# sevagh/umx.cpp

Hardware: AMD Instinct MI355X
Metric: realtime-factor (audio-sec/wall-sec) UMX-L 4-stem, 60 s seg (higher is better)
Workload: dtype f32 (activations as 2 x fp16 planes of the power-of-two-scaled row, integer weights exact in fp16, f32 accumulate on the fp16 matrix cores; fp32-grade: 1.4-2.2x the error of an fp32 evaluation, profiles/r06_v2_accuracy_vs_float64.txt)

## Files before the change

umx.cpp_amd/csrc/engine.hip:

```cpp
#include "../../include/umx_hip.h"
#include <chrono>
#include <dlfcn.h>

#include <algorithm>
#include <numeric>
#include <cmath>
#include <cstdio>
#include <cstdlib>
#include <cstring>
#include <map>
#include <mutex>
#include <string>
#include <vector>

#include "common.h"
#include "gemm_bf16x3.h"
#include "gemm_planes.h"
#include "gemm_planes_pp.h"
#include "gemm_planes_ps.h"
#include "lstm_kernels.h"
#include "lstm_batch.h"
#include "lstm_batch8.h"
#include "track_kernels.h"
#include "resample.h"
// ... 104 lines not shown
{
    static const RoctxApi api;
    if (!api.push)
        return;
    if (t_stage_range_open)
        api.pop();
    t_stage_range_open = stage >= 0 && stage < ST_COUNT;
    if (t_stage_range_open)
        api.push(api.names[stage]);
}
struct StageRangeCloser
{
    ~StageRangeCloser() { stage_range(-1); }
};
}

struct Lane
{
    TargetAct ta[4];
    float2 *spec = nullptr, *y = nullptr, *frames = nullptr;
    float *x = nullptr, *wpart = nullptr, *Rc = nullptr;
    unsigned *maxabs = nullptr;
};

struct Slot
{
    hipStream_t stream = nullptr;
    Lane lane[LSTMB_MAX_TRACKS];
    float *hbuf = nullptr;
    float *wv = nullptr;
    bool lstm_wrote_planes[3] = {false, false, false};
    bool lstm_rows_f32[3] = {true, true, true};
    unsigned *status = nullptr, *lsync = nullptr;
    unsigned long long *lprof = nullptr;
    hipEvent_t ev[ST_COUNT + 1] = {};
    hipEvent_t evk[ST_COUNT] = {};
    bool evk_set[ST_COUNT] = {};
    hipEvent_t rec_done[3] = {};
    hipEvent_t k_done = nullptr;
    hipEvent_t out_free = nullptr;
    bool out_free_valid = false;
    bool have_times = false, last_persistent = false, used = false;
};
}

namespace
{
struct LstmGate
{
    std::mutex m;
    struct Grid
    {
        hipEvent_t done;
        int units;
        hipStream_t stream;
        unsigned long long seq;
    };
    std::vector<Grid> inflight;
    std::vector<hipEvent_t> pool;
    unsigned long long seq = 0;
    int reserved = 0;
    std::vector<int> reservations;
};
LstmGate g_gate[16];

template <class Launch> hipError_t lstm_gate_launch(int device, hipStream_t st, int units, int capacity_units, Launch launch)
// ... 212 lines not shown
            slot[si].used = false;
    }
    int B = 1;
    bool lstm_batched = false;
    unsigned tag_epoch = 0;
    unsigned next_tag_base()
    {
        tag_epoch = (tag_epoch + 1) & 0xFFFFF;
        return tag_epoch << 12;
    }
    int cur = 0;
    long long nseg = 0;
    size_t lsync_words = 0;
    bool persistent_ok = true;
    int n_cus = 256;
    struct PendingCall
    {
        int nb;
        const float *audio[LSTMB_MAX_TRACKS];
        int n[LSTMB_MAX_TRACKS];
        float *out[4 * LSTMB_MAX_TRACKS];
        float *host_out[4 * LSTMB_MAX_TRACKS];
        const float *host_audio[LSTMB_MAX_TRACKS];
        unsigned flags;
    };
    static constexpr int kBackupCalls = 8;
    std::vector<PendingCall> pending;
    bool pending_lost = false;
    float *backup = nullptr;
    bool no_recovery = false, recovering = false;
    int recover();
    int lstm_poll_delay = 0;
    int env_gemm_ps = -1;
    int env_gemm_pp = -1;
    const char *gemm_kernel_last[4] = {"none", "none", "none", "none"};
    const char *lstm_kernel_last = "none";
    int lstm_capacity = 0;
    unsigned last_flags = 0;
    hipStream_t stream = nullptr;

    void set_error(const std::string &s) { err = s; }

    template <class T_> int dalloc(T_ **p, size_t count, bool zero = true)
    {
        void *q = nullptr;
        UMX_HIP_CHECK(hipMalloc(&q, std::max<size_t>(count, 1) * sizeof(T_)));
        allocs.push_back(q);
        if (zero)
            UMX_HIP_CHECK(hipMemset(q, 0, std::max<size_t>(count, 1) * sizeof(T_)));
        *p = reinterpret_cast<T_ *>(q);
        return UMX_OK;
    }
    template <class T_> int upload(T_ **p, const std::vector<T_> &h)
    {
        int rc = dalloc(p, h.size(), false);
        if (rc)
            return rc;
        UMX_HIP_CHECK(hipMemcpy(*p, h.data(), h.size() * sizeof(T_), hipMemcpyHostToDevice));
        return UMX_OK;
    }
    int init(int device_, int hidden, int segment_samples, const umx_tensor_view *tensors, int n_tensors,
             unsigned create_flags, int n_tracks);
    size_t weight_bytes = 0;
    bool wiener_fused = true;
    bool gemm_planes = false;
    void launch_split(Lane &ln, int nl, hipStream_t st, int which, const int *active, int nact);
    void launch_gemm_planes(Lane &ln, int nl, hipStream_t st, int mode, int layer, const int *active, int nact, bool dbg);
    void launch_gemm_lanes(Slot &sl, hipStream_t st, int nb, const float *const *audio_dev, int mode, int layer, const int *active,
                           int nact, bool dbg);
    bool u8_dequant = false;
    unsigned char *whh_q[3] = {};
    float whh_s[3][8] = {}, whh_o[3][8] = {};
    int infer_device(const float *audio_dev, int n, float *const out[4], unsigned flags);
    int infer_batch(int nb, const float *const *audio_dev, const int *n, float *const *out , unsigned flags);
    int lstm_batch_capacity = 0;
    bool lstm_batch8_ok = false;
    int lstm8_poll_delay = 0;
    bool env_lstm8_paired = true;
    int env_lstm8_min = 1;
    bool lstm_rowsums = false;
    bool lstm_writes_planes = false;
    size_t state_floats() const { return (size_t)4 * 12 * Hl; }
    struct TrackRequest
    {
        int n_tracks = 0;
        const float *const *audio = nullptr;
        const int *length = nullptr;
        const int *rate = nullptr;
        const int *shift_offset = nullptr;
        float *const *out = nullptr;
        unsigned flags = 0;
        void (*progress)(float, void *) = nullptr;
        void *progress_user = nullptr;
        bool ensemble = false;
        const MixSpec *mix = nullptr;
    };
    int tracks(const TrackRequest &rq);
    int tracks_once(const TrackRequest &rq);
    std::map<std::pair<int, int>, float *> rs_taps;
    int resample_plan(int rate_in, int rate_out, ResampleGeom &g, const float **taps_dev);
// ... 148 lines not shown
```

umx.cpp_amd/csrc/engine_init.h:

```cpp
namespace
{
bool dequant(const umx_tensor_view &tv, size_t expect, std::vector<float> &out)
{
    size_t nel = 1;
    for (int i = 0; i < tv.n_dims; ++i)
        nel *= (size_t)tv.ne[i];
    if (nel != expect)
        return false;
    out.resize(nel);
    if (tv.dtype == UMX_DTYPE_F32)
        memcpy(out.data(), tv.data, nel * sizeof(float));
    else if (tv.dtype == UMX_DTYPE_U8)
    {
        const uint8_t *q = static_cast<const uint8_t *>(tv.data);
        for (size_t i = 0; i < nel; ++i)
            out[i] = (float)q[i] * tv.scale + tv.offset;
    }
    else if (tv.dtype == UMX_DTYPE_U16)
    {
        const uint16_t *q = static_cast<const uint16_t *>(tv.data);
        for (size_t i = 0; i < nel; ++i)
            out[i] = (float)q[i] * tv.scale + tv.offset;
    }
    else
// ... 67 lines not shown
            return false;
        }
        return true;
    };

    const bool keepq = !(create_flags & UMX_CREATE_DEQUANTISE_AT_LOAD);
    auto view = [&](int tg, const std::string &name) -> const umx_tensor_view * {
        auto it = idx[tg].find(name);
        return it == idx[tg].end() ? nullptr : it->second;
    };
    auto all_q = [&](const std::string &name, int dtype, size_t expect) {
        for (int tg = 0; tg < 4; ++tg)
        {
            const umx_tensor_view *tv = view(tg, name);
            size_t n = 1;
            for (int i = 0; tv && i < tv->n_dims; ++i)
                n *= (size_t)tv->ne[i];
            if (!keepq || !tv || tv->dtype != dtype || n != expect)
                return false;
        }
        return true;
    };

    if (create_flags & UMX_CREATE_GEMM_F32)
    {
        set_error("UMX_CREATE_GEMM_F32: the fp32-MFMA GEMM flavour was removed in round 3 (slower and, against float64, less accurate "
                  "than the split-operand kernels: profiles/r02_accuracy_vs_float64.txt)");
        return UMX_ERR_ARG;
    }
    if (const char *e = getenv("UMX_GEMM_PP"))
        env_gemm_pp = atoi(e);
    if (const char *e = getenv("UMX_GEMM_PS"))
        env_gemm_ps = atoi(e);
    if (const char *e = getenv("UMX_LSTM8_POLL_DELAY"))
        lstm8_poll_delay = atoi(e);
    if (const char *e = getenv("UMX_LSTM8_PAIRED"))
        env_lstm8_paired = atoi(e) != 0;
    if (const char *e = getenv("UMX_LSTM8_MIN_LANES"))
        env_lstm8_min = atoi(e);
    if (const char *e = getenv("UMX_LSTM_POLL_DELAY"))
        lstm_poll_delay = atoi(e);
    wiener_fused = lstm_batched;
    if (const char *e = getenv("UMX_WIENER"))
        wiener_fused = std::string(e) == "fused";
    gemm_planes = (create_flags & UMX_CREATE_GEMM_PLANES) || (lstm_batched && !(create_flags & UMX_CREATE_GEMM_STAGED));
    Tp = gemm_planes ? std::max(T, 256) : round_up(T, 128);

    const int G = 4 * Hl;
    std::vector<int> gate_row(G);
    for (int sl = 0; sl < S; ++sl)
        for (int g = 0; g < 4; ++g)
            for (int u = 0; u < 16; ++u)
                gate_row[g * Hl + sl * 16 + u] = sl * 64 + u * 4 + g;
    std::vector<int> fc3_row(NOUT);
    for (int r = 0; r < NOUT; ++r)
        fc3_row[r] = r / NBINS * MAGP + r % NBINS;
    struct WeightDesc
    {
        std::string name[2];
        int nsrc, rows, cols, dst_rows, cols_pad;
        const std::vector<int> *dst_row;
        int dtype;
    };
    WeightDesc wd[W_COUNT];
    wd[W_FC1] = {{"fc1.weight"}, 1, H, NIN, H, KX, nullptr, UMX_DTYPE_U8};
    for (int l = 0; l < 3; ++l)
// ... 348 lines not shown
            }
        }
        {
            const WienerStrides ls = lane_strides();
            float2 *spec_all, *y_all, *frames_all;
            float *wpart_all, *Rc_all;
            unsigned *maxabs_all;
            if (int rc = dalloc(&spec_all, (size_t)B * ls.spec))
                return rc;
            if (int rc = dalloc(&y_all, (size_t)B * ls.y))
                return rc;
            if (int rc = dalloc(&frames_all, (size_t)B * ls.frames))
                return rc;
            if (int rc = dalloc(&wpart_all, (size_t)B * ls.part))
                return rc;
            if (int rc = dalloc(&Rc_all, (size_t)B * ls.rc))
                return rc;
            if (int rc = dalloc(&maxabs_all, (size_t)B))
                return rc;
            for (int ln = 0; ln < B; ++ln)
            {
                Lane &L = sl.lane[ln];
                L.x = x_all + (size_t)ln * Tp * KX;
                L.spec = spec_all + (size_t)ln * ls.spec;
                L.y = y_all + (size_t)ln * ls.y;
                L.frames = frames_all + (size_t)ln * ls.frames;
                L.wpart = wpart_all + (size_t)ln * ls.part;
                L.Rc = Rc_all + (size_t)ln * ls.rc;
                L.maxabs = maxabs_all + ln;
            }
        }
        if (int rc = dalloc(&sl.status, 4))
            return rc;
        if (int rc = dalloc(&sl.hbuf, (size_t)2 * 8 * Hl))
            return rc;
        if (int rc = dalloc(&sl.lsync, lsync_words))
            return rc;
        if (int rc = dalloc(&sl.lprof, 1024 + 64 * 8 * 5))
            return rc;
        for (int i = 0; i <= ST_COUNT; ++i)
            UMX_HIP_CHECK(hipEventCreate(&sl.ev[i]));
        for (int i : {ST_FC1, ST_IH0, ST_IH1, ST_IH2, ST_FC2, ST_FC3})
            UMX_HIP_CHECK(hipEventCreate(&sl.evk[i]));
        for (int l = 0; l < 3; ++l)
            UMX_HIP_CHECK(hipEventCreateWithFlags(&sl.rec_done[l], hipEventDisableTiming));
    }
    stream = slot[0].stream;
    {
        int cus = 0;
        UMX_HIP_CHECK(hipDeviceGetAttribute(&cus, hipDeviceAttributeMultiprocessorCount, device));
        n_cus = cus;
        const bool want8 = lstm_batched && B >= env_lstm8_min && !u8_dequant && whh_q[0] && whh_q[1] && whh_q[2];
        const LstmbLanes ll = lstmb_lanes(B);
        constexpr int kNone = 1 << 30;
        int per_cu[3] = {kNone, kNone, kNone};
        for (const LstmKernel &k : kLstmKernels)
        {
            if (k.hl != Hl || (k.family == LSTM_BATCH && !lstm_batched) || (k.family == LSTM_BATCH8 && !want8))
                continue;
            if (k.lds)
                UMX_HIP_CHECK(hipFuncSetAttribute(k.fn, hipFuncAttributeMaxDynamicSharedMemorySize, (int)k.lds));
            int v = 0;
            UMX_HIP_CHECK(hipOccupancyMaxActiveBlocksPerMultiprocessor(&v, k.fn, LSTM_THREADS, k.family == LSTM_BATCH ? lstmb_lds_bytes(ll.nbp, ll.bulk) : k.lds));
            per_cu[k.family] = std::min(per_cu[k.family], v);
        }
        lstm_capacity = per_cu[LSTM_PERSISTENT] == kNone ? 0 : per_cu[LSTM_PERSISTENT] * cus;
// ... 88 lines not shown
```

umx.cpp_amd/csrc/engine_stages.h:

```cpp
void umx_hip_ctx::launch_gemm(Lane &sl, hipStream_t st, int mode, int layer, const int *active, int nact, bool dbg)
{
    GemmArgs g;
    memset(&g, 0, sizeof g);
    g.M = Tp;
    g.T = T;
    int bq = BQ_F32;
    for (int i = 0; i < nact; ++i)
    {
        const TargetBufs &b = tb[active[i]];
        const TargetAct &c = sl.ta[active[i]];
        const GemmWeight &w = b.w[gemm_weight(mode, layer)];
        GemmTarget &t = g.t[i];
        switch (mode)
        {
        case G_FC1:
            t.A = sl.x; t.C = c.cat;
            t.e0 = b.bn1[0]; t.e1 = b.bn1[1]; t.e2 = b.bn1[2]; t.e3 = b.bn1[3];
            t.q0 = b.in_scale; t.q1 = b.in_mean;
            g.N = H; g.K = KX; g.lda = KX; g.ldc = 2 * H;
            break;
        case G_IH:
            t.A = layer == 0 ? c.cat : layer == 1 ? c.la : c.lb;
            t.C = c.P; t.e0 = b.ih_b[layer];
            g.N = 4 * H; g.K = H; g.lda = layer == 0 ? 2 * H : H; g.ldc = 4 * H;
// ... 51 lines not shown
        case SP_CATR:
            a.src[i] = c.cat + H; a.dst[i] = c.cat_p; a.rowsum[i] = lstm_rowsums ? nullptr : c.rs_catR;
            a.cols = H; a.ld_src = 2 * H; a.ld_dst = 2 * H; a.col0_dst = H; a.plane = rows_all * 2 * H;
            break;
        case SP_LA:
            a.src[i] = c.la; a.dst[i] = c.la_p; a.rowsum[i] = lstm_rowsums ? nullptr : c.rs_la;
            a.cols = H; a.ld_src = H; a.ld_dst = H; a.col0_dst = 0; a.plane = rows_all * H;
            break;
        case SP_LB:
            a.src[i] = c.lb; a.dst[i] = c.lb_p; a.rowsum[i] = lstm_rowsums ? nullptr : c.rs_lb;
            a.cols = H; a.ld_src = H; a.ld_dst = H; a.col0_dst = 0; a.plane = rows_all * H;
            break;
        default:
            a.src[i] = c.a2; a.dst[i] = c.a2_p; a.rowsum[i] = c.rs_a2; a.rowunscale[i] = c.rsc_a2;
            a.cols = H; a.ld_src = H; a.ld_dst = H; a.col0_dst = 0; a.plane = rows_all * H;
            break;
        }
    }
    a.rows_valid = nl * Tp;
    const dim3 grid(round_up(nl * Tp, 256) / 4, 1, nact);
    if (which == SP_XS && a.cols <= 3072)
    {
        hipLaunchKernelGGL(split_planes_shared_kernel<6>, dim3(grid.x), dim3(256), 0, st, a, nact);
        return;
    }
    if (a.cols <= 1024)
        hipLaunchKernelGGL(split_planes_kernel<2>, grid, dim3(256), 0, st, a);
    else if (a.cols <= 3072)
        hipLaunchKernelGGL(split_planes_kernel<6>, grid, dim3(256), 0, st, a);
    else
        hipLaunchKernelGGL(split_planes_kernel<8>, grid, dim3(256), 0, st, a);
}

void umx_hip_ctx::launch_gemm_planes(Lane &ln, int nl, hipStream_t st, int mode, int layer, const int *active, int nact, bool dbg)
{
    GemmPArgs g;
    memset(&g, 0, sizeof g);
    g.M = round_up(nl * Tp, 256);
    g.lanes = nl;
    g.T = T;
    g.Tp_lane = Tp;
    g.mag_lane = (size_t)2 * T * MAGP;
    g.a_unscale = 1.0f / (float)(1 << GP_SPLIT_FIXED_EXP);
    const size_t rows_all = (size_t)B * Tp + Mpad;
    int nbp = 2;
    for (int i = 0; i < nact; ++i)
    {
        const TargetBufs &b = tb[active[i]];
        const TargetAct &c = ln.ta[active[i]];
        const GemmWeight &w = b.w[gemm_weight(mode, layer)];
        GemmPTarget &t = g.t[i];
        t.bsplit = 0x7fffffff;
        switch (mode)
        {
        case G_FC1:
            t.A = c.xs_p; t.C = c.cat; t.rs0 = c.rs_xs; t.rsc = c.rsc_xs;
            t.e0 = b.bn1[0]; t.e1 = b.bn1[1]; t.e2 = b.bn1[2]; t.e3 = b.bn1[3];
            g.N = H; g.K = KX; g.lda = KX; g.ldc = 2 * H; g.a_plane = rows_all * KX;
            break;
        case G_IH:
            t.A = layer == 0 ? c.cat_p : layer == 1 ? c.la_p : c.lb_p;
            t.rs0 = layer == 0 ? c.rs_catL : layer == 1 ? c.rs_la : c.rs_lb;
            if (layer > 0 && lstm_rowsums)
                t.rs1 = t.rs0 + rows_all;
            t.C = c.P; t.e0 = b.ih_b[layer];
            t.bsplit = 2 * H;
            g.N = 4 * H; g.K = H; g.lda = layer == 0 ? 2 * H : H; g.ldc = 4 * H;
            g.a_plane = layer == 0 ? rows_all * 2 * H : rows_all * H;
            break;
        case G_FC2:
            t.A = c.cat_p; t.C = c.a2; t.rs0 = c.rs_catL; t.rs1 = c.rs_catR;
            if (lstm_rowsums)
                t.rs2 = c.rs_catR + rows_all;
            t.e0 = b.bn2[0]; t.e1 = b.bn2[1]; t.e2 = b.bn2[2]; t.e3 = b.bn2[3];
            g.N = H; g.K = 2 * H; g.lda = 2 * H; g.ldc = H; g.a_plane = rows_all * 2 * H;
            break;
        default:
            t.A = c.a2_p; t.C = c.mag; t.rs0 = c.rs_a2; t.rsc = c.rsc_a2;
            t.e0 = b.bn3[0]; t.e1 = b.bn3[1]; t.e2 = b.bn3[2]; t.e3 = b.bn3[3];
            t.q0 = b.out_scale; t.q1 = b.out_mean;
            g.N = NOUT_PAD; g.K = H; g.lda = H; g.ldc = 0; g.a_plane = rows_all * H;
            break;
        }
        t.B = static_cast<const unsigned short *>(w.p);
        t.bs[0] = w.s[0]; t.bs[1] = w.s[1];
        t.bo2[0] = w.o[0]; t.bo2[1] = w.o[1];
        nbp = w.form;
    }
    const int blocks_big = (g.N / 256) * (g.M / 256) * nact;
    const bool big = g.N % 256 == 0 && blocks_big >= 224;
    const int bm = big ? 256 : 128;
    const int gemm_pp = env_gemm_pp;
    const bool pp = big && (gemm_pp < 0 || ((gemm_pp >> mode) & 1));
    const int ps_wgs = n_cus / 8 * 8;
    const bool ps = pp && (env_gemm_ps < 0 || ((env_gemm_ps >> mode) & 1)) && g.K / GP_BK >= 6 && ps_wgs >= 8 && blocks_big > ps_wgs && g.Tp_lane >= 256;
    gemm_kernel_last[mode] = ps ? "gemm_planes_ps_kernel" : pp ? "gemm_planes_pp_kernel" : "gemm_planes_kernel";
    const GemmKernel k = gp_kernel(mode, nbp, ps ? GP_PS : pp ? GP_PP : big ? GP_256 : GP_128);
    void *kargs[] = {&g, &nact};
    if (ps)
        (void)hipLaunchKernel(k.fn, dim3(ps_wgs), dim3(512), kargs, k.lds, st);
    else
        (void)hipLaunchKernel(k.fn, dim3((unsigned)round_up((g.N / bm) * (g.M / bm), 8), 1, nact), dim3(pp ? 512 : big ? 1024 : 256), kargs,
                              k.lds, st);
}

void umx_hip_ctx::launch_gemm_lanes(Slot &sl, hipStream_t st, int nb, const float *const *audio_dev, int mode, int layer,
                                    const int *active, int nact, bool dbg)
{
    if (nact <= 0)
        return;
    for (int l0 = 0; l0 < nb;)
    {
        if (!audio_dev[l0])
        {
            ++l0;
            continue;
        }
        int l1 = l0 + 1;
        while (gemm_planes && l1 < nb && audio_dev[l1])
            ++l1;
        if (gemm_planes)
        {
            const int which = mode == G_FC1 ? SP_XS : mode == G_IH ? (layer == 0 ? SP_CATL : layer == 1 ? SP_LA : SP_LB) : mode == G_FC2 ? SP_CATR : SP_A2;
            const int from_layer = which == SP_LA ? 0 : which == SP_LB ? 1 : which == SP_CATR ? 2 : -1;
            if (from_layer < 0 || !sl.lstm_wrote_planes[from_layer])
                launch_split(sl.lane[l0], l1 - l0, st, which, active, nact);
            {
                const int stg = mode == G_FC1 ? ST_FC1 : mode == G_IH ? ST_IH0 + 2 * layer : mode == G_FC2 ? ST_FC2 : ST_FC3;
                sl.evk_set[stg] = sl.evk[stg] && hipEventRecord(sl.evk[stg], st) == hipSuccess;
            }
            launch_gemm_planes(sl.lane[l0], l1 - l0, st, mode, layer, active, nact, dbg);
        }
        else
            launch_gemm(sl.lane[l0], st, mode, layer, active, nact, dbg);
        l0 = l1;
    }
}

int umx_hip_ctx::stage_front(Slot &sl, hipStream_t st, int nb, const float *const *audio_dev, const int *n, const int *active,
                             int nact)
{
    stage_range(ST_STFT);
    for (int i = 0; i < ST_COUNT; ++i)
        sl.evk_set[i] = false;
    UMX_HIP_CHECK(hipEventRecord(sl.ev[ST_STFT], st));
    {
        StftIn in;
        in.lanes = lane_set(nb, audio_dev);
        for (int i = 0; i < in.lanes.count; ++i)
        {
            in.audio[i] = audio_dev[in.lanes.id[i]];
            in.n[i] = n[in.lanes.id[i]];
        }
        Lane &L0 = sl.lane[0];
        UMX_HIP_CHECK(hipMemsetAsync(L0.maxabs, 0, sizeof(unsigned) * B, st));
        hipLaunchKernelGGL(stft_kernel, dim3((T + STFT_RUN - 1) / STFT_RUN, in.lanes.count), dim3(256), 0, st, in, N, T, window, tw1, tw2, L0.spec, lane_strides().spec, L0.x,
                           (size_t)Tp * KX, L0.maxabs);
    }
    stage_range(ST_FC1);
    UMX_HIP_CHECK(hipEventRecord(sl.ev[ST_FC1], st));
    launch_gemm_lanes(sl, st, nb, audio_dev, G_FC1, 0, active, nact, false);
    stage_range(ST_IH0);
    UMX_HIP_CHECK(hipEventRecord(sl.ev[ST_IH0], st));
    launch_gemm_lanes(sl, st, nb, audio_dev, G_IH, 0, active, nact, false);
// ... 312 lines not shown
```

umx.cpp_amd/csrc/gemm_planes.h:

```cpp
#pragma once
#include "gemm_bf16x3.h"
#include <cmath>
#include <cstring>

namespace umx
{

struct GemmPTarget
{
    const unsigned short *A;
    const unsigned short *B;
    float *C;
    const float *e0, *e1, *e2, *e3, *q0, *q1;
    const float *rs0, *rs1, *rs2;
    const float *rsc;
    float bs[2], bo2[2];
    int bsplit;
};

struct GemmPArgs
{
    GemmPTarget t[4];
    int M, N, K, lda, ldc, T;
    size_t a_plane;
    float a_unscale;
    int Tp_lane;
    int lanes;
    size_t mag_lane;
};

constexpr int GP_BK = 32;
constexpr int GP_SPLIT_FIXED_EXP = 14;
__host__ __device__ constexpr int gp_stage_bytes(int WM, int WN, int NBP) { return (2 * 64 * WM + NBP * 64 * WN) * 64; }
__host__ __device__ constexpr int gp_stages(int WM, int WN, int NBP)
{
    return 3 * gp_stage_bytes(WM, WN, NBP) <= (WM * WN >= 16 ? 160 : 80) * 1024 ? 3 : 2;
}
__host__ __device__ constexpr int gp_lds_bytes(int WM, int WN, int NBP) { return gp_stages(WM, WN, NBP) * gp_stage_bytes(WM, WN, NBP); }


struct SplitArgs
{
    const float *src[4];
    unsigned short *dst[4];
    float *rowsum[4];
    float *rowunscale[4];
    const float *scale[4], *mean[4];
    int T, Tp, cols, ld_src, ld_dst, col0_dst;
    int rows_valid;
    size_t plane;
};

typedef _Float16 f16x8 __attribute__((ext_vector_type(8)));

__device__ __forceinline__ void split2_f16(const float (&x)[8], float scale, uint4 &p1, uint4 &p2)
{
    f16x8 h1, h2;
#pragma unroll
    for (int j = 0; j < 8; ++j)
    {
        const float v = x[j] * scale;
// ... 390 lines not shown
```

umx.cpp_amd/csrc/gemm_planes_ps.h:

```cpp
#pragma once
#include "gemm_planes_pp.h"

namespace umx
{

typedef float floatx4 __attribute__((ext_vector_type(4)));
typedef unsigned int v4u32 __attribute__((ext_vector_type(4)));
constexpr int PS_TAB_ROWS = 4, PS_TAB_COLS = 8;
__host__ __device__ constexpr int ps_lds_bytes(int NBP) { return gp_lds_bytes(4, 4, NBP) + (PS_TAB_ROWS + PS_TAB_COLS) * 256 * 4; }
constexpr unsigned PS_DROP = 0x40000000u;
#ifndef PS_STORE_AUX
#define PS_STORE_AUX 2
#endif
#ifndef PS_PREWAIT
#define PS_PREWAIT 1
#endif
#ifndef PS_A_AUX
#define PS_A_AUX 0
#endif
#ifndef PS_B_AUX
#define PS_B_AUX 0
#endif
#ifndef PS_PROFILE
#define PS_PROFILE 0
#endif

template <int MODE, int NBP> __global__ __launch_bounds__(512, 1) void gemm_planes_ps_kernel(GemmPArgs args, int ntg)
{
    extern __shared__ __attribute__((aligned(16))) unsigned char gp_smem[];
    constexpr int MI = 4, BM = 256, BN = 256, KKP = 2;
    constexpr int A_PL = BM * 64, B_PL = BN * 64;
    constexpr int BUF_BYTES = 2 * A_PL + NBP * B_PL, STAGES = gp_stages(4, 4, NBP);
    static_assert(NBP == 1 || NBP == 2, "weight planes: 1 (u8) or 2 (u16, fp32)");
    float *const rowtab = reinterpret_cast<float *>(gp_smem + STAGES * BUF_BYTES);
    float *const coltab = rowtab + PS_TAB_ROWS * 256;
    const int tid = threadIdx.x, lane = tid & 63, wave = __builtin_amdgcn_readfirstlane(tid >> 6);
    const int grp = wave >> 2, ws = wave & 3;
    const int wm = grp, wn = ws, lr = lane & 31, lh = lane >> 5;
    const int K = args.K, lda = args.lda, nk = K / GP_BK;

    const int gx = args.N / BN, gy = args.M / BM, total = gx * gy, total_all = total * ntg;
    const int wpx = (int)gridDim.x >> 3, chunk = (total_all + 7) >> 3;
    const int v_begin = (int)(blockIdx.x & 7) * chunk + (int)(blockIdx.x >> 3), v_end = min(((int)(blockIdx.x & 7) + 1) * chunk, total_all);
    if (v_begin >= v_end)
        return;
    const int ntiles = (v_end - v_begin + wpx - 1) / wpx, ntrips = ntiles * nk;
#define PS_DECODE(v_, TGI, M0, N0, LN0, F0)                                                                          \
    {                                                                                                                \
        const int tg_ = (v_) / total, vt_ = (v_) - tg_ * total;                                                      \
        const int per_group_ = GEMM_GROUP_M * gx, group_ = vt_ / per_group_, first_m_ = group_ * GEMM_GROUP_M;       \
        const int gsize_ = min(gy - first_m_, GEMM_GROUP_M), in_group_ = vt_ - group_ * per_group_;                  \
        const int q_ = in_group_ / gsize_;                                                                           \
        TGI = tg_;                                                                                                   \
        M0 = (first_m_ + in_group_ - q_ * gsize_) * BM;                                                              \
        N0 = q_ * BN;                                                                                                \
        if (MODE == G_FC3)                                                                                           \
        {                                                                                                            \
            LN0 = M0 / args.Tp_lane;                                                                                 \
            F0 = M0 - LN0 * args.Tp_lane;                                                                            \
        }                                                                                                            \
    }

    typedef __attribute__((address_space(3))) void *lds_ptr;
    const int st_chunk = (lane & 3) ^ ((lane >> 4) & 3);
    const int voffA = ((lane >> 2) * lda) * 2 + st_chunk * 16, voffB = ((lane >> 2) * K) * 2 + st_chunk * 16;
    const unsigned lds0 = (unsigned)(size_t)(lds_ptr)gp_smem;
    constexpr bool BOTH = PP_DMA_BOTH && STAGES == 3;
    constexpr int DEAL = BOTH ? 8 : 4, PER = 16 / DEAL;
    constexpr int A_GROUPS = 2 * (BM / 16), B_GROUPS = NBP * (BN / 16), NA = A_GROUPS / DEAL, NB = B_GROUPS / DEAL, DMA_PER_WAVE = NA + NB;
    static_assert(DMA_PER_WAVE <= 16 && A_GROUPS % DEAL == 0 && B_GROUPS % DEAL == 0 && BM == 256 && BN == 256, "vmcnt bookkeeping below");
    const int w8 = (BOTH ? 4 * grp : 0) + ws;
    const bool issuer = grp == 0 || BOTH;
    const unsigned lds_w = lds0 + (unsigned)w8 * 1024u;
    int a_it[NA], b_it[NB];
#pragma unroll
    for (int it = 0; it < NA; ++it)
        a_it[it] = (int)((long)(it / PER) * (long)args.a_plane * 2) + (it % PER) * DEAL * 32 * lda;
#pragma unroll
    for (int it = 0; it < NB; ++it)
        b_it[it] = (int)((long)(it / PER) * (long)args.N * K * 2) + (it % PER) * DEAL * 32 * K;
    int d_tile = 0, d_k = 0, koff = 0, a_tile, b_tile, n_tgi, n_m0, n_n0, n_ln0 = 0, n_f0 = 0;
    PS_DECODE(v_begin, n_tgi, n_m0, n_n0, n_ln0, n_f0)
    __amdgpu_buffer_rsrc_t rsA = __builtin_amdgcn_make_buffer_rsrc(const_cast<unsigned short *>(args.t[n_tgi].A), 0, 0x7fffffff, 0x00020000);
    __amdgpu_buffer_rsrc_t rsB = __builtin_amdgcn_make_buffer_rsrc(const_cast<unsigned short *>(args.t[n_tgi].B), 0, 0x7fffffff, 0x00020000);
    a_tile = (int)((long)(n_m0 + 16 * w8) * lda * 2);
    b_tile = (int)((long)(n_n0 + 16 * w8) * K * 2);
    int c_tgi = n_tgi, c_m0 = n_m0, c_n0 = n_n0, c_ln0 = n_ln0, c_f0 = n_f0;
#define PS_DMA_ISSUE(buf)                                                                                            \
    {                                                                                                                \
        const unsigned lb_ = lds_w + (unsigned)((buf)*BUF_BYTES);                                                    \
        const int ao_ = a_tile + koff, bo_ = b_tile + koff;                                                          \
        _Pragma("unroll") for (int it = 0; it < NA; ++it)                                                            \
        {                                                                                                            \
            const int so_ = ao_ + a_it[it];                                                                          \
            __builtin_amdgcn_raw_ptr_buffer_load_lds(rsA, (lds_ptr)(size_t)(lb_ + (it / PER) * A_PL + (it % PER) * DEAL * 1024), 16, voffA, so_, 0, PS_A_AUX); \
        }                                                                                                            \
        _Pragma("unroll") for (int it = 0; it < NB; ++it)                                                            \
        {                                                                                                            \
            const int so_ = bo_ + b_it[it];                                                                          \
            __builtin_amdgcn_raw_ptr_buffer_load_lds(rsB, (lds_ptr)(size_t)(lb_ + 2 * A_PL + (it / PER) * B_PL + (it % PER) * DEAL * 1024), 16, voffB, so_, 0, PS_B_AUX); \
        }                                                                                                            \
    }
#define PS_DMA_ADVANCE()                                                                                             \
    {                                                                                                                \
        koff += 2 * GP_BK;                                                                                           \
        if (++d_k == nk)                                                                                             \
        {                                                                                                            \
            d_k = 0;                                                                                                 \
            koff = 0;                                                                                                \
            if (++d_tile < ntiles)                                                                                   \
            {                                                                                                        \
                PS_DECODE(v_begin + d_tile * wpx, n_tgi, n_m0, n_n0, n_ln0, n_f0)                                    \
                rsA = __builtin_amdgcn_make_buffer_rsrc(const_cast<unsigned short *>(args.t[n_tgi].A), 0, 0x7fffffff, 0x00020000); \
                rsB = __builtin_amdgcn_make_buffer_rsrc(const_cast<unsigned short *>(args.t[n_tgi].B), 0, 0x7fffffff, 0x00020000); \
                a_tile = (int)((long)(n_m0 + 16 * w8) * lda * 2);                                                    \
                b_tile = (int)((long)(n_n0 + 16 * w8) * K * 2);                                                      \
            }                                                                                                        \
        }                                                                                                            \
    }

    floatx16 acc[MI][2];
    const floatx16 zero16 = {0.f, 0.f, 0.f, 0.f, 0.f, 0.f, 0.f, 0.f, 0.f, 0.f, 0.f, 0.f, 0.f, 0.f, 0.f, 0.f};
    const int sw = (lr >> 2) & 3;
    const int fragA = (wm * 32 * MI + lr) * 64, fragB = 2 * A_PL + (wn * 64 + lr) * 64;
    f16x8 fa[2][MI][KKP], fb[NBP][2][KKP];
#define PS_LD(off) (*reinterpret_cast<const f16x8 *>(gp_smem + (off)))
#define PS_LOAD_KL(buf, kl)                                                                                          \
    {                                                                                                                \
        const int bo = (buf)*BUF_BYTES;                                                                              \
        const int co = (((kl)*2 + lh) ^ sw) * 16;                                                                    \
        _Pragma("unroll") for (int p = 0; p < NBP; ++p)                                                              \
        {                                                                                                            \
            fb[p][0][kl] = PS_LD(bo + fragB + p * B_PL + co);                                                        \
            fb[p][1][kl] = PS_LD(bo + fragB + p * B_PL + 32 * 64 + co);                                              \
        }                                                                                                            \
        _Pragma("unroll") for (int p = 1; p >= 0; --p)                                                               \
            _Pragma("unroll") for (int mi = 0; mi < MI; ++mi)                                                        \
                fa[p][mi][kl] = PS_LD(bo + fragA + p * A_PL + mi * 32 * 64 + co);                                    \
    }
#define PS_MFMA(A, B, C) __builtin_amdgcn_mfma_f32_32x32x16_f16(A, B, C, 0, 0, 0)
#define PS_BAND(mi, kl, ZERO)                                                                                        \
    {                                                                                                                \
        acc[mi][0] = PS_MFMA(fa[1][mi][kl], fb[0][0][kl], (ZERO) ? zero16 : acc[mi][0]);                             \
        acc[mi][1] = PS_MFMA(fa[1][mi][kl], fb[0][1][kl], (ZERO) ? zero16 : acc[mi][1]);                             \
        if (NBP == 2)                                                                                                \
// ... 150 lines not shown
#define PS_TAB_FINISH()                                                                                              \
    {                                                                                                                \
        if (grp == 0)                                                                                                \
        {                                                                                                            \
            const GemmPTarget &tg_ = args.t[e_tgi];                                                                  \
            const int sel_ = e_n0 >= tg_.bsplit ? 1 : 0;                                                             \
            const float rsc_ = tg_.rsc ? rowtab[tid] : args.a_unscale, r0_ = rowtab[256 + tid];                      \
            const float r1_ = tg_.rs1 ? rowtab[512 + tid] : 0.f, r2_ = tg_.rs2 ? rowtab[768 + tid] : 0.f;            \
            unsigned off_ = (unsigned)tid * ldc4;                        \
            if (MODE == G_FC3)                                                                                       \
            {                                                                                                        \
                                                      \
                const int f1_ = e_f0 + tid, second_ = f1_ >= args.Tp_lane ? 1 : 0, f_ = f1_ - second_ * args.Tp_lane; \
                off_ = f_ < args.T ? ((unsigned)second_ * (unsigned)args.mag_lane + (unsigned)f_ * MAGP) * 4u : PS_DROP; \
            }                                                                                                        \
            rowtab[tid] = tg_.bs[sel_] * rsc_;                            \
            rowtab[256 + tid] = tg_.bo2[sel_] * (tg_.rs2 ? (r0_ + r1_) + r2_ : tg_.rs1 ? r0_ + r1_ : r0_);           \
            reinterpret_cast<unsigned *>(rowtab)[512 + tid] = off_;                                                  \
            if (MODE != G_IH)                                                                                        \
            {                                                                                                        \
                const float sd_ = sqrtf(coltab[256 + tid] + 1e-5f);                         \
                coltab[256 + tid] = sd_;                                                                             \
                coltab[2 * 256 + tid] = 1.0f / sd_;                                                                  \
            }                                                                                                        \
            if (MODE == G_FC3)                                                                                       \
            {                                                                                                        \
                          \
                const int n_ = e_n0 + tid, ch_ = n_ >= MAGP ? 1 : 0, bin_ = n_ - ch_ * MAGP;                         \
                reinterpret_cast<unsigned *>(coltab)[7 * 256 + tid] = bin_ < NBINS ? ((unsigned)(ch_ * args.T) * MAGP + (unsigned)bin_) * 4u : PS_DROP; \
            }                                                                                                        \
        }                                                                                                            \
    }

    int cur = 0, u = 0;
#define PS_M(FIRST, LATE, YOUNG1, TAB, FINISH, SPLIT)                                                                       \
    {                                                                                                                \
        const int nxt_ = STAGES == 3 ? (cur == 0 ? 2 : cur - 1) : cur ^ 1;  \
        const bool more_ = u + STAGES - 1 < ntrips, late_ = (LATE) && grp == 0;                                      \
        if ((TAB) && issuer)                                                                                         \
            PS_TAB_RAW()                                                                                             \
        if (more_ && !late_)                                                                                         \
        {                                                                                                            \
            if (issuer)                                                                                              \
                PS_DMA_ISSUE(nxt_)                                                                                   \
            PS_DMA_ADVANCE()                                                                                         \
        }                                                                                                            \
        PS_LOAD_KL(cur, 0)                                                                                           \
        if (!(FIRST))                                                                                                \
            PS_LOAD_KL(cur, 1)                                                                                       \
        if (FINISH)                                                                                                  \
            PS_TAB_FINISH()                                                                                          \
        PS_WAIT_LDS();                                                                                               \
        if (BOTH && grp == 1 && u + 1 < ntrips)                                                                      \
        {                                                                                                            \
             \
            if (YOUNG1)                                                                                              \
            {                                                                                                        \
                if (!PS_PREWAIT)                                                                                     \
                    PS_WAIT_VM(63);                                                                                  \
            }                                                                                                        \
            else if (u + 2 < ntrips)                                                                                 \
                PS_WAIT_VM(DMA_PER_WAVE);                                                                            \
            else                                                                                                     \
                PS_WAIT_VM(0);                                                                                       \
        }                                                                                                            \
        if (!(SPLIT) || grp == 0)              \
            PS_BARRIER()                                                                                             \
        if (more_ && late_)                                                                                          \
        {                                                                                                            \
            PS_DMA_ISSUE(nxt_)                                                                                       \
            PS_DMA_ADVANCE()                                                                                         \
        }                                                                                                            \
    }
#define PS_C_END(YOUNG0)                                                                                             \
    {                                                                                                                \
        if (grp == 0 && u + 1 < ntrips)                                                                              \
        {                                                                                                            \
            if (YOUNG0)                                                                                              \
            {                                                                                                        \
                if (!PS_PREWAIT)                                                                                     \
                    PS_WAIT_VM(63);                                                                                  \
            }                                                                                                        \
            else if (STAGES == 3 && u + 2 < ntrips)                                                                  \
                PS_WAIT_VM(DMA_PER_WAVE);                                                                            \
            else                                                                                                     \
                PS_WAIT_VM(0);                                                                                       \
        }                                                                                                            \
        PS_BARRIER()                                                                                                 \
        cur = cur + 1 == STAGES ? 0 : cur + 1;                                                                       \
        ++u;                                                                                                         \
    }
#define PS_C_FIRST_TAIL()                                                                                            \
    {                                                                                                                \
        PS_LOAD_KL(cur, 1)                                                                                           \
        PS_WAIT_LDS();                                                                                               \
        PS_STEP(1)                                                                                                   \
    }

    const int tab_trip = nk - 3;
    {
        if (issuer)
            PS_DMA_ISSUE(0)
        PS_DMA_ADVANCE()
        if (STAGES == 3)
        {
            if (issuer)
                PS_DMA_ISSUE(1)
            PS_DMA_ADVANCE()
            if (issuer)
                PS_WAIT_VM(DMA_PER_WAVE);
        }
        else if (issuer)
            PS_WAIT_VM(0);
    }
    PS_BARRIER()
    if (grp == 1)
        PS_BARRIER()
    PS_M(true, false, false, false, false, false)
    __builtin_amdgcn_s_setprio(1);
#pragma unroll
    for (int mi = 0; mi < MI; ++mi)
        PS_BAND(mi, 0, true)
    PS_C_FIRST_TAIL()
    __builtin_amdgcn_s_setprio(0);
    PS_C_END(false)
    [[maybe_unused]] long long pq_loop = 0, pq_epi = 0, pq_epi_m = 0, pq_t0 = 0, pq_t1 = 0, pq_t2 = 0;
    const long long pq_start = PS_PROFILE ? clock64() : 0;
    for (int tile = 0; tile < ntiles; ++tile)
    {
        if (PS_PROFILE)
            pq_t0 = clock64();
        for (int kt = 1; kt < nk; ++kt)
        {
            const bool tab = kt == tab_trip;
            PS_M(false, kt == 1, tile > 0 && kt == 1, tab, false, false)
            __builtin_amdgcn_s_setprio(1);
            PS_STEP(0)
            PS_STEP(1)
            __builtin_amdgcn_s_setprio(0);
            PS_C_END(tile > 0 && kt == 1 && STAGES == 3)
        }
        if (PS_PROFILE)
        {
            pq_t1 = clock64();
            pq_loop += pq_t1 - pq_t0;
        }
        e_m0 = c_m0;
        e_n0 = c_n0;
        e_tgi = c_tgi;
        e_ln0 = c_ln0;
        e_f0 = c_f0;
        if (tile + 1 < ntiles)
        {
            c_m0 = n_m0;
            c_n0 = n_n0;
            c_tgi = n_tgi;
            c_ln0 = n_ln0;
            c_f0 = n_f0;
            PS_M(true, false, false, false, true, true)
            if (PS_PROFILE)
            {
                pq_t2 = clock64();
                pq_epi_m += pq_t2 - pq_t1;
            }
            if (PS_PREWAIT && issuer)
                PS_WAIT_VM(0);
            PS_EPI_SETUP()
#pragma unroll
            for (int mi = 0; mi < MI; ++mi)
                PS_EPI_BAND(mi)
            if (grp == 1)
                PS_BARRIER()
            __builtin_amdgcn_s_setprio(1);
#pragma unroll
            for (int mi = 0; mi < MI; ++mi)
                PS_BAND(mi, 0, true)
            PS_C_FIRST_TAIL()
            __builtin_amdgcn_s_setprio(0);
            PS_C_END(true)
            if (PS_PROFILE)
                pq_epi += clock64() - pq_t2;
        }
    }
    if (PS_PROFILE && (blockIdx.x == 8 || blockIdx.x == 101) && (tid == 0 || tid == 256))
        printf("# ps<%d,%d> wg %d wave %d tiles %d trips/tile %d: cycles  normal trip %lld  first trip: M phase %lld, C phase with the epilogue %lld  per tile %lld\n", MODE, NBP,
               (int)blockIdx.x, wave, ntiles, nk, pq_loop / ((long long)ntiles * (nk - 1)), pq_epi_m / max(ntiles - 1, 1), pq_epi / max(ntiles - 1, 1),
               (clock64() - pq_start) / ntiles);
    if (grp == 0)
        PS_BARRIER()
    PS_TAB_FINISH()
    PS_BARRIER()
    PS_EPI_SETUP()
#pragma unroll
    for (int mi = 0; mi < MI; ++mi)
        PS_EPI_BAND(mi)
#undef PS_M
#undef PS_C_END
#undef PS_C_FIRST_TAIL
#undef PS_DECODE
#undef PS_DMA_ISSUE
#undef PS_DMA_ADVANCE
#undef PS_LD
#undef PS_LOAD_KL
#undef PS_MFMA
#undef PS_BAND
#undef PS_TERM
#undef PS_STEP
#undef PS_WAIT_VM
#undef PS_WAIT_LDS
#undef PS_BARRIER
#undef PS_EPI_ROWS
#undef PS_EPI_BAND
#undef PS_EPI_SETUP
#undef PS_TAB_PIECE
#undef PS_TAB_RAW
#undef PS_TAB_FINISH
}

}
```

Before: 38570.

## Replace static tile split in persistent GEMM with atomic work-stealing walk

The persistent split-plane GEMM kernel previously gave each workgroup a fixed strided set of tiles within its XCC-aligned chunk. It now claims tiles dynamically through per-chunk atomic counters and steals from the other chunks once its own chunk is drained. The next tile is claimed during the current tile's epilogue so the prefetch pipeline keeps running. The aim is to balance tail imbalance across workgroups and XCCs, at the cost of a memset and atomics per launch, with some risk of losing L2 locality when tiles are stolen across chunks.

```diff
diff --git a/umx.cpp_amd/csrc/engine.hip b/umx.cpp_amd/csrc/engine.hip
--- a/umx.cpp_amd/csrc/engine.hip
+++ b/umx.cpp_amd/csrc/engine.hip
@@ -160,6 +160,7 @@
     bool lstm_wrote_planes[3] = {false, false, false};
     bool lstm_rows_f32[3] = {true, true, true};
     unsigned *status = nullptr, *lsync = nullptr;
+    unsigned *gemm_walk = nullptr;
     unsigned long long *lprof = nullptr;
     hipEvent_t ev[ST_COUNT + 1] = {};
     hipEvent_t evk[ST_COUNT] = {};
@@ -438,6 +439,7 @@
     int recover();
     int lstm_poll_delay = 0;
     int env_gemm_ps = -1;
+    bool env_gemm_ps_walk = true;
     int env_gemm_pp = -1;
     const char *gemm_kernel_last[4] = {"none", "none", "none", "none"};
     const char *lstm_kernel_last = "none";
@@ -471,7 +473,7 @@
     bool wiener_fused = true;
     bool gemm_planes = false;
     void launch_split(Lane &ln, int nl, hipStream_t st, int which, const int *active, int nact);
-    void launch_gemm_planes(Lane &ln, int nl, hipStream_t st, int mode, int layer, const int *active, int nact, bool dbg);
+    void launch_gemm_planes(Lane &ln, int nl, hipStream_t st, int mode, int layer, const int *active, int nact, bool dbg, unsigned *walk);
     void launch_gemm_lanes(Slot &sl, hipStream_t st, int nb, const float *const *audio_dev, int mode, int layer, const int *active,
                            int nact, bool dbg);
     bool u8_dequant = false;
diff --git a/umx.cpp_amd/csrc/engine_init.h b/umx.cpp_amd/csrc/engine_init.h
--- a/umx.cpp_amd/csrc/engine_init.h
+++ b/umx.cpp_amd/csrc/engine_init.h
@@ -123,6 +123,8 @@
         env_gemm_pp = atoi(e);
     if (const char *e = getenv("UMX_GEMM_PS"))
         env_gemm_ps = atoi(e);
+    if (const char *e = getenv("UMX_GEMM_PS_WALK"))
+        env_gemm_ps_walk = atoi(e) != 0;
     if (const char *e = getenv("UMX_LSTM8_POLL_DELAY"))
         lstm8_poll_delay = atoi(e);
     if (const char *e = getenv("UMX_LSTM8_PAIRED"))
@@ -537,6 +539,8 @@
         }
         if (int rc = dalloc(&sl.status, 4))
             return rc;
+        if (int rc = dalloc(&sl.gemm_walk, 8))
+            return rc;
         if (int rc = dalloc(&sl.hbuf, (size_t)2 * 8 * Hl))
             return rc;
         if (int rc = dalloc(&sl.lsync, lsync_words))
diff --git a/umx.cpp_amd/csrc/engine_stages.h b/umx.cpp_amd/csrc/engine_stages.h
--- a/umx.cpp_amd/csrc/engine_stages.h
+++ b/umx.cpp_amd/csrc/engine_stages.h
@@ -107,7 +107,7 @@
         hipLaunchKernelGGL(split_planes_kernel<8>, grid, dim3(256), 0, st, a);
 }
 
-void umx_hip_ctx::launch_gemm_planes(Lane &ln, int nl, hipStream_t st, int mode, int layer, const int *active, int nact, bool dbg)
+void umx_hip_ctx::launch_gemm_planes(Lane &ln, int nl, hipStream_t st, int mode, int layer, const int *active, int nact, bool dbg, unsigned *walk)
 {
     GemmPArgs g;
     memset(&g, 0, sizeof g);
@@ -173,7 +173,11 @@
     const GemmKernel k = gp_kernel(mode, nbp, ps ? GP_PS : pp ? GP_PP : big ? GP_256 : GP_128);
     void *kargs[] = {&g, &nact};
     if (ps)
+    {
+        if (env_gemm_ps_walk && walk && hipMemsetAsync(walk, 0, 8 * sizeof(unsigned), st) == hipSuccess)
+            g.walk = walk;
         (void)hipLaunchKernel(k.fn, dim3(ps_wgs), dim3(512), kargs, k.lds, st);
+    }
     else
         (void)hipLaunchKernel(k.fn, dim3((unsigned)round_up((g.N / bm) * (g.M / bm), 8), 1, nact), dim3(pp ? 512 : big ? 1024 : 256), kargs,
                               k.lds, st);
@@ -204,7 +208,7 @@
                 const int stg = mode == G_FC1 ? ST_FC1 : mode == G_IH ? ST_IH0 + 2 * layer : mode == G_FC2 ? ST_FC2 : ST_FC3;
                 sl.evk_set[stg] = sl.evk[stg] && hipEventRecord(sl.evk[stg], st) == hipSuccess;
             }
-            launch_gemm_planes(sl.lane[l0], l1 - l0, st, mode, layer, active, nact, dbg);
+            launch_gemm_planes(sl.lane[l0], l1 - l0, st, mode, layer, active, nact, dbg, sl.gemm_walk);
         }
         else
             launch_gemm(sl.lane[l0], st, mode, layer, active, nact, dbg);
diff --git a/umx.cpp_amd/csrc/gemm_planes.h b/umx.cpp_amd/csrc/gemm_planes.h
--- a/umx.cpp_amd/csrc/gemm_planes.h
+++ b/umx.cpp_amd/csrc/gemm_planes.h
@@ -27,6 +27,7 @@
     int Tp_lane;
     int lanes;
     size_t mag_lane;
+    unsigned *walk;
 };
 
 constexpr int GP_BK = 32;
diff --git a/umx.cpp_amd/csrc/gemm_planes_ps.h b/umx.cpp_amd/csrc/gemm_planes_ps.h
--- a/umx.cpp_amd/csrc/gemm_planes_ps.h
+++ b/umx.cpp_amd/csrc/gemm_planes_ps.h
@@ -7,7 +7,7 @@
 typedef float floatx4 __attribute__((ext_vector_type(4)));
 typedef unsigned int v4u32 __attribute__((ext_vector_type(4)));
 constexpr int PS_TAB_ROWS = 4, PS_TAB_COLS = 8;
-__host__ __device__ constexpr int ps_lds_bytes(int NBP) { return gp_lds_bytes(4, 4, NBP) + (PS_TAB_ROWS + PS_TAB_COLS) * 256 * 4; }
+__host__ __device__ constexpr int ps_lds_bytes(int NBP) { return gp_lds_bytes(4, 4, NBP) + (PS_TAB_ROWS + PS_TAB_COLS) * 256 * 4 + 16; }
 constexpr unsigned PS_DROP = 0x40000000u;
 #ifndef PS_STORE_AUX
 #define PS_STORE_AUX 2
@@ -23,6 +23,30 @@
 #endif
 #ifndef PS_PROFILE
 #define PS_PROFILE 0
+#endif
+
+#if PS_PROFILE
+__device__ long long ps_walk_rec[512][8];
+__device__ unsigned ps_walk_done;
+__device__ __noinline__ void ps_walk_record(int mode, int nbp, int tiles, long long s0, long long s1, long long r0, long long r1, long long q1, long long q2, long long q3)
+{
+    unsigned xcc = 0;
+    asm volatile("s_getreg_b32 %0, hwreg(HW_REG_XCC_ID)" : "=s"(xcc));
+    volatile long long *r = ps_walk_rec[blockIdx.x & 511];
+    r[0] = (long long)(xcc & 15u) | ((long long)tiles << 8);
+    r[1] = s0, r[2] = s1, r[3] = r0, r[4] = r1, r[5] = q1, r[6] = q2, r[7] = q3;
+    __threadfence();
+    if (__hip_atomic_fetch_add(&ps_walk_done, 1u, __ATOMIC_ACQ_REL, __HIP_MEMORY_SCOPE_AGENT) != gridDim.x - 1)
+        return;
+    __hip_atomic_store(&ps_walk_done, 0u, __ATOMIC_RELAXED, __HIP_MEMORY_SCOPE_AGENT);
+    __threadfence();
+    for (unsigned b = 0; b < gridDim.x && b < 512; ++b)
+    {
+        volatile long long *q = ps_walk_rec[b];
+        printf("# psw<%d,%d> wg %u xcc %d tiles %d shader %lld %lld real %lld %lld quarters %lld %lld %lld\n", mode, nbp, b, (int)(q[0] & 15), (int)(q[0] >> 8), q[1], q[2],
+               q[3], q[4], q[5], q[6], q[7]);
+    }
+}
 #endif
 
 template <int MODE, int NBP> __global__ __launch_bounds__(512, 1) void gemm_planes_ps_kernel(GemmPArgs args, int ntg)
@@ -41,10 +65,64 @@
 
     const int gx = args.N / BN, gy = args.M / BM, total = gx * gy, total_all = total * ntg;
     const int wpx = (int)gridDim.x >> 3, chunk = (total_all + 7) >> 3;
-    const int v_begin = (int)(blockIdx.x & 7) * chunk + (int)(blockIdx.x >> 3), v_end = min(((int)(blockIdx.x & 7) + 1) * chunk, total_all);
-    if (v_begin >= v_end)
+    const bool dyn = args.walk != nullptr;
+    constexpr unsigned PS_NONE = 0x7fffffffu;
+    unsigned *const claim_lds = reinterpret_cast<unsigned *>(coltab + PS_TAB_COLS * 256);
+    const auto claimed_tile = [&](unsigned ticket) -> unsigned {
+        unsigned cx = claim_lds[1] & 7u;
+        for (;;)
+        {
+            const int b = (int)cx * chunk, e = min(b + chunk, total_all);
+            if (ticket < (unsigned)max(e - b, 0))
+            {
+                claim_lds[1] = cx;
+                return (unsigned)b + ticket;
+            }
+            if (((cx + 1) & 7u) == (blockIdx.x & 7u))
+            {
+                claim_lds[1] = cx;
+                return PS_NONE;
+            }
+            cx = (cx + 1) & 7u;
+            ticket = __hip_atomic_fetch_add(args.walk + cx, 1u, __ATOMIC_RELAXED, __HIP_MEMORY_SCOPE_AGENT);
+        }
+    };
+    int c_v, next_v, v_end;
+    if (dyn)
+    {
+        if (tid == 0)
+        {
+            claim_lds[1] = blockIdx.x & 7;
+            claim_lds[2] = claimed_tile(__hip_atomic_fetch_add(args.walk + (blockIdx.x & 7), 1u, __ATOMIC_RELAXED, __HIP_MEMORY_SCOPE_AGENT));
+            claim_lds[0] = claim_lds[2] == PS_NONE
+                               ? PS_NONE
+                               : claimed_tile(__hip_atomic_fetch_add(args.walk + (claim_lds[1] & 7u), 1u, __ATOMIC_RELAXED, __HIP_MEMORY_SCOPE_AGENT));
+        }
+        __syncthreads();
+        v_end = total_all;
+        c_v = __builtin_amdgcn_readfirstlane((int)claim_lds[2]);
+        next_v = __builtin_amdgcn_readfirstlane((int)claim_lds[0]);
+    }
+    else
+    {
+        v_end = min(((int)(blockIdx.x & 7) + 1) * chunk, total_all);
+        c_v = (int)(blockIdx.x & 7) * chunk + (int)(blockIdx.x >> 3);
+        next_v = c_v + wpx;
+    }
+    if (c_v >= v_end)
+    {
+#if PS_PROFILE
+        if (tid == 0)
+            ps_walk_record(MODE, NBP, 0, 0, 0, wall_clock64(), wall_clock64(), 0, 0, 0);
+#endif
         return;
-    const int ntiles = (v_end - v_begin + wpx - 1) / wpx, ntrips = ntiles * nk;
+    }
+    bool has_next = next_v < v_end;
+    int tile = 0, tiles_known = has_next ? 2 : 1;
+    int kt = 0;
+#define PS_MORE(d_) (kt + (d_) < nk || has_next)
+    [[maybe_unused]] const int pw_nt = max((chunk + wpx - 1) / wpx, 1);
+    [[maybe_unused]] const long long pw_s0 = PS_PROFILE ? clock64() : 0, pw_r0 = PS_PROFILE ? wall_clock64() : 0;
 #define PS_DECODE(v_, TGI, M0, N0, LN0, F0)                                                                          \
     {                                                                                                                \
         const int tg_ = (v_) / total, vt_ = (v_) - tg_ * total;                                                      \
@@ -79,8 +157,8 @@
 #pragma unroll
     for (int it = 0; it < NB; ++it)
         b_it[it] = (int)((long)(it / PER) * (long)args.N * K * 2) + (it % PER) * DEAL * 32 * K;
-    int d_tile = 0, d_k = 0, koff = 0, a_tile, b_tile, n_tgi, n_m0, n_n0, n_ln0 = 0, n_f0 = 0;
-    PS_DECODE(v_begin, n_tgi, n_m0, n_n0, n_ln0, n_f0)
+    int d_k = 0, koff = 0, a_tile, b_tile, n_tgi, n_m0, n_n0, n_ln0 = 0, n_f0 = 0;
+    PS_DECODE(c_v, n_tgi, n_m0, n_n0, n_ln0, n_f0)
     __amdgpu_buffer_rsrc_t rsA = __builtin_amdgcn_make_buffer_rsrc(const_cast<unsigned short *>(args.t[n_tgi].A), 0, 0x7fffffff, 0x00020000);
     __amdgpu_buffer_rsrc_t rsB = __builtin_amdgcn_make_buffer_rsrc(const_cast<unsigned short *>(args.t[n_tgi].B), 0, 0x7fffffff, 0x00020000);
     a_tile = (int)((long)(n_m0 + 16 * w8) * lda * 2);
@@ -108,9 +186,9 @@
         {                                                                                                            \
             d_k = 0;                                                                                                 \
             koff = 0;                                                                                                \
-            if (++d_tile < ntiles)                                                                                   \
-            {                                                                                                        \
-                PS_DECODE(v_begin + d_tile * wpx, n_tgi, n_m0, n_n0, n_ln0, n_f0)                                    \
+            if (has_next)                                           \
+            {                                                                                                        \
+                PS_DECODE(next_v, n_tgi, n_m0, n_n0, n_ln0, n_f0)                                                    \
                 rsA = __builtin_amdgcn_make_buffer_rsrc(const_cast<unsigned short *>(args.t[n_tgi].A), 0, 0x7fffffff, 0x00020000); \
                 rsB = __builtin_amdgcn_make_buffer_rsrc(const_cast<unsigned short *>(args.t[n_tgi].B), 0, 0x7fffffff, 0x00020000); \
                 a_tile = (int)((long)(n_m0 + 16 * w8) * lda * 2);                                                    \
@@ -327,13 +405,16 @@
         }                                                                                                            \
     }
 
-    int cur = 0, u = 0;
+    int cur = 0;
+    unsigned claim_r = 0;
 #define PS_M(FIRST, LATE, YOUNG1, TAB, FINISH, SPLIT)                                                                       \
     {                                                                                                                \
         const int nxt_ = STAGES == 3 ? (cur == 0 ? 2 : cur - 1) : cur ^ 1;  \
-        const bool more_ = u + STAGES - 1 < ntrips, late_ = (LATE) && grp == 0;                                      \
+        const bool more_ = PS_MORE(STAGES - 1), late_ = (LATE) && grp == 0;                                          \
         if ((TAB) && issuer)                                                                                         \
             PS_TAB_RAW()                                                                                             \
+        if ((FINISH) && dyn && tid == 0)  \
+            claim_r = __hip_atomic_fetch_add(args.walk + (claim_lds[1] & 7u), 1u, __ATOMIC_RELAXED, __HIP_MEMORY_SCOPE_AGENT); \
         if (more_ && !late_)                                                                                         \
         {                                                                                                            \
             if (issuer)                                                                                              \
@@ -346,7 +427,7 @@
         if (FINISH)                                                                                                  \
             PS_TAB_FINISH()                                                                                          \
         PS_WAIT_LDS();                                                                                               \
-        if (BOTH && grp == 1 && u + 1 < ntrips)                                                                      \
+        if (BOTH && grp == 1 && PS_MORE(1))                                                                          \
         {                                                                                                            \
              \
             if (YOUNG1)                                                                                              \
@@ -354,7 +435,7 @@
                 if (!PS_PREWAIT)                                                                                     \
                     PS_WAIT_VM(63);                                                                                  \
             }                                                                                                        \
-            else if (u + 2 < ntrips)                                                                                 \
+            else if (PS_MORE(2))                                                                                     \
                 PS_WAIT_VM(DMA_PER_WAVE);                                                                            \
             else                                                                                                     \
                 PS_WAIT_VM(0);                                                                                       \
@@ -369,21 +450,20 @@
     }
 #define PS_C_END(YOUNG0)                                                                                             \
     {                                                                                                                \
-        if (grp == 0 && u + 1 < ntrips)                                                                              \
+        if (grp == 0 && PS_MORE(1))                                                                                  \
         {                                                                                                            \
             if (YOUNG0)                                                                                              \
             {                                                                                                        \
                 if (!PS_PREWAIT)                                                                                     \
                     PS_WAIT_VM(63);                                                                                  \
             }                                                                                                        \
-            else if (STAGES == 3 && u + 2 < ntrips)                                                                  \
+            else if (STAGES == 3 && PS_MORE(2))                                                                      \
                 PS_WAIT_VM(DMA_PER_WAVE);                                                                            \
             else                                                                                                     \
                 PS_WAIT_VM(0);                                                                                       \
         }                                                                                                            \
         PS_BARRIER()                                                                                                 \
         cur = cur + 1 == STAGES ? 0 : cur + 1;                                                                       \
-        ++u;                                                                                                         \
     }
 #define PS_C_FIRST_TAIL()                                                                                            \
     {                                                                                                                \
@@ -421,13 +501,29 @@
     PS_C_END(false)
     [[maybe_unused]] long long pq_loop = 0, pq_epi = 0, pq_epi_m = 0, pq_t0 = 0, pq_t1 = 0, pq_t2 = 0;
     const long long pq_start = PS_PROFILE ? clock64() : 0;
-    for (int tile = 0; tile < ntiles; ++tile)
+    [[maybe_unused]] long long pw_q1 = 0, pw_q2 = 0, pw_q3 = 0;
+    for (; tile < tiles_known; ++tile)
     {
         if (PS_PROFILE)
+        {
             pq_t0 = clock64();
-        for (int kt = 1; kt < nk; ++kt)
+            if (tile == pw_nt / 4)
+                pw_q1 = wall_clock64();
+            if (tile == pw_nt / 2)
+                pw_q2 = wall_clock64();
+            if (tile == pw_nt * 3 / 4)
+                pw_q3 = wall_clock64();
+        }
+        for (kt = 1; kt < nk; ++kt)
         {
             const bool tab = kt == tab_trip;
+            if (kt == 2)
+            {
+                if (dyn)
+                    next_v = __builtin_amdgcn_readfirstlane((int)claim_lds[0]);
+                has_next = next_v < v_end;
+                tiles_known = tile + (has_next ? 2 : 1);
+            }
             PS_M(false, kt == 1, tile > 0 && kt == 1, tab, false, false)
             __builtin_amdgcn_s_setprio(1);
             PS_STEP(0)
@@ -445,8 +541,12 @@
         e_tgi = c_tgi;
         e_ln0 = c_ln0;
         e_f0 = c_f0;
-        if (tile + 1 < ntiles)
+        if (tile + 1 < tiles_known)
         {
+            kt = 0;
+            if (!dyn)
+                next_v += wpx;
+            claim_r = 0;
             c_m0 = n_m0;
             c_n0 = n_n0;
             c_tgi = n_tgi;
@@ -460,6 +560,8 @@
             }
             if (PS_PREWAIT && issuer)
                 PS_WAIT_VM(0);
+            if (dyn && tid == 0)
+                claim_lds[0] = claimed_tile(claim_r);
             PS_EPI_SETUP()
 #pragma unroll
             for (int mi = 0; mi < MI; ++mi)
@@ -477,10 +579,10 @@
                 pq_epi += clock64() - pq_t2;
         }
     }
-    if (PS_PROFILE && (blockIdx.x == 8 || blockIdx.x == 101) && (tid == 0 || tid == 256))
+    if (PS_PROFILE == 1 && (blockIdx.x == 8 || blockIdx.x == 101) && (tid == 0 || tid == 256))
         printf("# ps<%d,%d> wg %d wave %d tiles %d trips/tile %d: cycles  normal trip %lld  first trip: M phase %lld, C phase with the epilogue %lld  per tile %lld\n", MODE, NBP,
-               (int)blockIdx.x, wave, ntiles, nk, pq_loop / ((long long)ntiles * (nk - 1)), pq_epi_m / max(ntiles - 1, 1), pq_epi / max(ntiles - 1, 1),
-               (clock64() - pq_start) / ntiles);
+               (int)blockIdx.x, wave, tile, nk, pq_loop / ((long long)tile * (nk - 1)), pq_epi_m / max(tile - 1, 1), pq_epi / max(tile - 1, 1),
+               (clock64() - pq_start) / tile);
     if (grp == 0)
         PS_BARRIER()
     PS_TAB_FINISH()
@@ -489,7 +591,17 @@
 #pragma unroll
     for (int mi = 0; mi < MI; ++mi)
         PS_EPI_BAND(mi)
+    if (PS_PROFILE)
+    {
+        PS_WAIT_VM(0);
+#if PS_PROFILE
+        const long long s1_ = clock64(), r1_ = wall_clock64();
+        if (tid == 0)
+            ps_walk_record(MODE, NBP, tile, pw_s0, s1_, pw_r0, r1_, pw_q1, pw_q2, pw_q3);
+#endif
+    }
 #undef PS_M
+#undef PS_MORE
 #undef PS_C_END
 #undef PS_C_FIRST_TAIL
 #undef PS_DECODE
```

After: 38870, median of 6. No clear change (+0.8%).
